# APRIL-ZJU/Ctrl-VIO

Measured on AMD Instinct MI355X. Metric: sliding-window solves/sec (10 KF, 200 lm, 2000 IMU), higher is better.
Workload: dtype f64; 1 GPU; config2: 10 KF / 200 landmarks / 2000 IMU sliding window (K = 24 knots, 814 reprojection blocks), <= 15 LM iterations (Ceres 1.14 trust region + projected line search); distinct_windows_per_gpu=64, streams_per_gpu=4, concurrent_solves_per_gpu=2

## Files before the change

### ctrl-vio_amd/csrc/kernels_solve.hpp

```cpp
#pragma once

namespace ctv {

__device__ __forceinline__ void begin_iteration(const Dev &d, int w, int *s_go) {
  Lm &lm = d.lm[w];
  if (threadIdx.x == 0) {
    int go = 0;
    if (!lm.status) {
      if (lm.ls_active) atomicAdd(d.n_active, 1);
      else if (lm.iter >= d.prm.max_iters) lm.status = 1 + 0;
      else if (lm.last_ok && __longlong_as_double((long long)lm.gmax_bits) <= d.prm.gtol) lm.status = 1 + 1;
      else if (lm.mu <= d.prm.min_radius) lm.status = 1 + 4;
      else {
        lm.iter += 1;
        lm.accept = 0; lm.step_valid = 0; lm.chol_fail = 0; lm.alpha = 1.0;
        atomicAdd(d.n_active, 1);
        go = 1;
      }
    }
    *s_go = go;
  }
  __syncthreads();
  if (!*s_go) return;
  const WinMeta &m = d.wins[w];
  const double mu = lm.mu;
  const double *Hd = d.HppS[lm.cur] + m.H0, *Hl = d.HllS[lm.cur] + m.lm0;
  for (int j = threadIdx.x; j < m.N; j += blockDim.x) {
    const bool act = d.active[m.u0 + j] != 0;
    const double c = d.cscale[m.u0 + j];
    const double h = (j < m.P) ? Hd[(long long)j * m.ldh + j] : Hl[j - m.P];
    const double sc = fmin(fmax(c * c * h, d.prm.min_diag), d.prm.max_diag);
    const double dd = act ? sc / (mu * c * c) : 0.0;
    d.dd[m.u0 + j] = dd;
    if (j >= m.P) {
      const int row = m.lm0 + d.lm_pos[m.lm0 + j - m.P];
      d.dinv[row] = (act && (h + dd) > 0.0) ? 1.0 / (h + dd) : 0.0;
      d.grs[row] = d.gS[lm.cur][m.u0 + j];
    }
  }
}
__global__ __launch_bounds__(256) void k_begin_iter(Dev d) {
  __shared__ int s_go;
  begin_iteration(d, blockIdx.x, &s_go);
}

__device__ __forceinline__ void tile_decode(int t, int &bi, int &bj) {
  bi = 0;
  while ((bi + 1) * (bi + 2) / 2 <= t) ++bi;
  bj = t - bi * (bi + 1) / 2;
}

struct SchurTiles {
  const int &K6, &P;
  __device__ bool nz_row(int b) const { return (16 * b < K6) || (P >= 16 * b && P - 1 < 16 * b + 16); }
  __device__ bool nz_col(int b) const { return (16 * b < K6) || (P - 1 >= 16 * b && P - 1 < 16 * b + 16); }
};

__device__ __forceinline__ void schur_row_range(const Dev &d, const WinMeta &m, int bi, int bj, int &lbeg, int &lend) {
  int rb = d.tl_beg[m.tr0 + bi], re = d.tl_end[m.tr0 + bi];
  if (16 * bi <= m.P && m.P < 16 * bi + 16) { rb = 0; re = m.Lobs; }
  lbeg = max(rb, d.tl_beg[m.tr0 + bj]);
  lend = min(re, d.tl_end[m.tr0 + bj]);
}

template <int NPRE, int NTQ> __global__ __launch_bounds__(512, NTQ <= 7 ? 4 : 2) void k_schur_window_f64(Dev d) {
  const int w = blockIdx.x;
  if (d.lm[w].status || d.lm[w].ls_active) return;
  const WinMeta &m = d.wins[w];
  const int P = m.P, L = m.L, ldw = m.ldw, u0 = m.u0, K6 = 6 * m.K, ldh = m.ldh;
  const int nt = ldw >> 4, ntile = nt * (nt + 1) / 2;
  extern __shared__ __attribute__((aligned(16))) double smd64[];
  const int ldl = ldw + 16;
  double *Wb = smd64;
  double *acts = Wb + 2 * 16 * ldl;
  double *ddv = acts + ldw;
  double *gv = ddv + ldw;
  double *dch = gv + ldw;
  int *tlist = reinterpret_cast<int *>(dch + 32);
  int &tcount = tlist[8 * NTQ];
  const int tid = threadIdx.x, wave = __builtin_amdgcn_readfirstlane(tid >> 6), lane = tid & 63, q4 = lane >> 4, l15 = lane & 15;
  const double *Wp = d.WS[d.lm[w].cur] + m.W0;
  const double *dinv = d.dinv + m.lm0, *gl = d.grs + m.lm0;
  for (int c = tid; c < ldw; c += 512) {
    const int cc = min(c, P - 1);
    acts[c] = (c < P && d.active[u0 + cc]) ? 1.0 : 0.0; ddv[c] = d.dd[u0 + cc]; gv[c] = d.gS[d.lm[w].cur][u0 + cc];
  }
  if (tid == 0) tcount = 0;
  const SchurTiles tiles{K6, P};
  __syncthreads();
  for (int t = tid; t < ntile; t += 512) {
    int ti, tj;
    tile_decode(t, ti, tj);
    if (tiles.nz_row(ti) && tiles.nz_col(tj)) { const int pos = atomicAdd(&tcount, 1); if (pos < 8 * NTQ) tlist[pos] = (ti << 8) | tj; }
  }
  const int nchunk = (m.Lobs + 15) >> 4, nel = 16 * ldl, NC = K6 + 2, nelc = 16 * NC;
  for (int e = tid; e < 2 * nel; e += 512) Wb[e] = 0.0;
  double pre[NPRE];
  double pre_d = 0.0;
  int pre_lc[NPRE];
  double keep[NPRE];
#pragma unroll
  for (int k = 0; k < NPRE; ++k) {
    const int e = min(tid + 512 * k, nelc - 1), cc = e % NC, c = cc < K6 ? cc : P - 1 + (cc - K6);
    pre_lc[k] = ((e / NC) << 16) | c | ((tid + 512 * k < nelc && c == P) ? 1 << 30 : 0);
  }
  auto fetch = [&](int ch) {
#pragma unroll
    for (int k = 0; k < NPRE; ++k) {
      const int l = min(16 * ch + ((pre_lc[k] >> 16) & 0xff), L - 1), c = pre_lc[k] & 0xffff;
      pre[k] = (c == P) ? gl[l] : Wp[(long long)l * ldw + c];
    }
    if (tid < 16) pre_d = dinv[min(16 * ch + tid, L - 1)];
  };
  auto stash = [&](int ch, int buf) {
#pragma unroll
    for (int k = 0; k < NPRE; ++k) {
      const int lr = (pre_lc[k] >> 16) & 0xff, c = pre_lc[k] & 0xffff;
      const bool lv = 16 * ch + lr < L && (pre_lc[k] >> 30) != 0;
      if (tid + 512 * k < nelc) Wb[buf * nel + lr * ldl + c] = lv ? pre[k] : 0.0;
    }
    if (tid < 16) dch[16 * buf + tid] = (16 * ch + tid < L) ? pre_d : 0.0;
  };
  __syncthreads();
#pragma unroll
  for (int k = 0; k < NPRE; ++k) keep[k] = acts[min(pre_lc[k] & 0xffff, ldw - 1)];
#pragma unroll
  for (int k = 0; k < NPRE; ++k) pre_lc[k] |= (tid + 512 * k < nelc && keep[k] != 0.0) ? 1 << 30 : 0;
  const int nact = min(tcount, 8 * NTQ);
  long long *dbg = (d.dbg && w == (d.nwin > 1000 ? 1000 : 0)) ? d.dbg + 96 : nullptr;
  int dbi = 0;
  CTV_STAMP(dbg, dbi, 30, tid == 0);
  int tij[NTQ];
#pragma unroll
  for (int q = 0; q < NTQ; ++q) tij[q] = __builtin_amdgcn_readfirstlane(tlist[(wave + 8 * q < nact) ? wave + 8 * q : min(wave, max(nact - 1, 0))]);
#pragma unroll
  for (int q = 0; q < NTQ; ++q) {
    int lb, le;
    schur_row_range(d, m, tij[q] >> 8, tij[q] & 255, lb, le);
    const bool real = wave + 8 * q < nact && le > lb;
    const int cb = real ? min(lb >> 4, 254) : 0, ce = real ? min((le + 15) >> 4, 255) : 0;
    tij[q] = __builtin_amdgcn_readfirstlane(tij[q] | (cb << 16) | (ce << 24));
  }
  const double *H = d.HppS[d.lm[w].cur] + m.H0;
  f64x4 acc[NTQ];
  const int opq = opaque_zero();
#pragma unroll
  for (int q = 0; q < NTQ; ++q) {
    const int tq = (tij[q] & 0xffff) + opq, jc = min(16 * (tq & 255) + l15, P - 1);
#pragma unroll
    for (int r = 0; r < 4; ++r) {
      const int ii = 16 * (tq >> 8) + q4 + 4 * r, ic = min(ii, P - 1);
      const double h = H[(unsigned)(ic * ldh + min(jc, ic))];
      acc[q][r] = ii < P ? -h : 0.0;
    }
  }
  if (nchunk > 0) { fetch(0); stash(0, 0); }
  __syncthreads();
  CTV_STAMP(dbg, dbi, 30, tid == 0);
  for (int ch = 0; ch < nchunk && nact > 0; ++ch) {
    const int buf = ch & 1;
    if (ch + 1 < nchunk) fetch(ch + 1);
    const double *B = Wb + buf * nel + q4 * ldl + l15;
    double dl[4];
#pragma unroll
    for (int s = 0; s < 4; ++s) dl[s] = dch[16 * buf + 4 * s + q4];
#pragma unroll
    for (int q = 0; q < NTQ; ++q) {
      { const int cb = (tij[q] >> 16) & 255, ce = (tij[q] >> 24) & 255; if (ch < cb || (ch >= ce && ce != 255)) continue; }
      double a[4], b[4];
#pragma unroll
      for (int s = 0; s < 4; ++s) {
        a[s] = B[4 * s * ldl + 16 * ((tij[q] >> 8) & 255)];
        b[s] = B[4 * s * ldl + 16 * (tij[q] & 255)];
      }
      __builtin_amdgcn_sched_barrier(0);
#pragma unroll
      for (int s = 0; s < 4; ++s) acc[q] = __builtin_amdgcn_mfma_f64_16x16x4f64(a[s], b[s] * dl[s], acc[q], 0, 0, 0);
      __builtin_amdgcn_sched_barrier(0);
    }
    if (ch + 1 < nchunk) stash(ch + 1, buf ^ 1);
    __syncthreads();
  }
  CTV_STAMP(dbg, dbi, 30, tid == 0);
  double *S = d.S + m.H0, *rhs = d.rhs + m.p0;
  auto pin = [](double &x) { asm volatile("" : "+v"(x)); };
  auto store_tile = [&](int ti, int tj, const double (&hs)[4], const double (&bs)[4]) {
    const int jj = 16 * tj + l15, jc = min(jj, P - 1);
    double a_j = acts[jc], dd_j = ddv[jc], g_j = gv[jc], a_i[4];
#pragma unroll
    for (int r = 0; r < 4; ++r) a_i[r] = acts[min(16 * ti + q4 + 4 * r, P - 1)];
    pin(a_j); pin(dd_j); pin(g_j);
#pragma unroll
    for (int r = 0; r < 4; ++r) pin(a_i[r]);
    const bool act_j = a_j != 0.0;
#pragma unroll
    for (int r = 0; r < 4; ++r) {
      const int ii = 16 * ti + q4 + 4 * r;
      if (ii < P && jj <= ii) {
        const bool on = a_i[r] != 0.0 && act_j;
        S[(long long)ii * ldh + jj] = on ? hs[r] + (ii == jj ? dd_j : 0.0) : (ii == jj ? 1.0 : 0.0);
      } else if (ii == P && jj < P) {
        rhs[jj] = act_j ? bs[r] - g_j : 0.0;
      }
    }
  };
#pragma unroll
  for (int q = 0; q < NTQ; ++q) {
    if (wave + 8 * q >= nact) continue;
    double hs[4], bs[4];
#pragma unroll
    for (int r = 0; r < 4; ++r) { hs[r] = -acc[q][r]; bs[r] = acc[q][r]; }
    store_tile((tij[q] >> 8) & 255, tij[q] & 255, hs, bs);
  }
  CTV_STAMP(dbg, dbi, 30, tid == 0);
  auto next_plain = [&](int t) {
    for (; t < ntile; t += 8) {
      int ti, tj;
      tile_decode(t, ti, tj);
      if (!(tiles.nz_row(ti) && tiles.nz_col(tj))) break;
    }
    return t;
  };
  if (d.schur_plain_in_H) {
    for (int c = tid; c < P; c += 512)
      if (!tiles.nz_col(c >> 4)) rhs[c] = acts[c] != 0.0 ? -gv[c] : 0.0;
  } else
  for (int tp = next_plain(wave); tp < ntile;) {
    int pi[4], pj[4];
#pragma unroll
    for (int u = 0; u < 4; ++u) {
      pi[u] = -1; pj[u] = 0;
      if (tp < ntile) { tile_decode(tp, pi[u], pj[u]); tp = next_plain(tp + 8); }
    }
    double hv[4][4];
#pragma unroll
    for (int u = 0; u < 4; ++u) {
      const int ti = max(pi[u], 0), jc = min(16 * pj[u] + l15, P - 1);
#pragma unroll
      for (int r = 0; r < 4; ++r) {
        const int ic = min(16 * ti + q4 + 4 * r, P - 1);
        hv[u][r] = H[(unsigned)(ic * ldh + min(jc, ic))];
      }
    }
    const double zero[4] = {0.0, 0.0, 0.0, 0.0};
#pragma unroll
    for (int u = 0; u < 4; ++u)
      if (pi[u] >= 0) store_tile(pi[u], pj[u], hv[u], zero);
  }
  CTV_STAMP(dbg, dbi, 30, tid == 0);
}

__global__ __launch_bounds__(64) void k_schur_tile_f64(Dev d, int ntile_max) {
  const int xcd = blockIdx.x & 7, slot = blockIdx.x >> 3;
  const int w = (slot / ntile_max) * 8 + xcd, tile = slot % ntile_max;
  if (w >= d.nwin) return;
  if (d.lm[w].status || d.lm[w].ls_active) return;
  const WinMeta &m = d.wins[w];
  const int P = m.P, L = m.L, ldw = m.ldw, u0 = m.u0, ldh = m.ldh;
  const int nt = P / 16 + 1;
  if (tile >= nt * (nt + 1) / 2) return;
  int bi, bj;
  tile_decode(tile, bi, bj);
  if (bj < d.env_first[m.tr0 + bi]) return;
  const int lane = threadIdx.x, q4 = lane >> 4, l15 = lane & 15;
  const int i = min(16 * bi + l15, ldw - 1), j = min(16 * bj + l15, ldw - 1);
  const bool rhs_lane = 16 * bi + l15 == P;
  const double ai = (16 * bi + l15 < P && d.active[u0 + min(i, P - 1)]) ? 1.0 : 0.0;
  const double aj = (16 * bj + l15 < P && d.active[u0 + min(j, P - 1)]) ? 1.0 : 0.0;
  const double *Wp = d.WS[d.lm[w].cur] + m.W0;
  const double *dinv = d.dinv + m.lm0, *gl = d.grs + m.lm0;
  int lbeg, lend;
  schur_row_range(d, m, bi, bj, lbeg, lend);
  f64x4 acc = {0.0, 0.0, 0.0, 0.0};
  for (int l0 = lbeg; l0 < lend; l0 += 16) {
    double wa[4], wb[4], dv[4], gv[4];
#pragma unroll
    for (int s = 0; s < 4; ++s) {
      const int lc = min(l0 + 4 * s + q4, L - 1);
      wa[s] = Wp[(long long)lc * ldw + i];
      wb[s] = Wp[(long long)lc * ldw + j];
      dv[s] = dinv[lc];
      gv[s] = gl[lc];
    }
#pragma unroll
    for (int s = 0; s < 4; ++s) wa[s] = rhs_lane ? gv[s] : wa[s] * ai;
#pragma unroll
    for (int s = 0; s < 4; ++s) {
      const bool lv = l0 + 4 * s + q4 < lend;
      acc = __builtin_amdgcn_mfma_f64_16x16x4f64(wa[s], lv ? wb[s] * aj * dv[s] : 0.0, acc, 0, 0, 0);
    }
  }
  double *S = d.S + m.H0, *rhs = d.rhs + m.p0;
  const double *H = d.HppS[d.lm[w].cur] + m.H0;
  const int jj = 16 * bj + l15, jc = min(jj, P - 1);
  const bool act_j = d.active[u0 + jc] != 0;
  const double dd_j = d.dd[u0 + jc], g_j = d.gS[d.lm[w].cur][u0 + jc];
  double hv[4];
  unsigned char act_i[4];
#pragma unroll
  for (int r = 0; r < 4; ++r) {
    const int ic = min(16 * bi + q4 + 4 * r, P - 1);
    act_i[r] = d.active[u0 + ic];
    hv[r] = H[(long long)ic * ldh + min(jc, ic)];
  }
#pragma unroll
  for (int r = 0; r < 4; ++r) {
    const int ii = 16 * bi + q4 + 4 * r;
    if (ii < P && jj <= ii) {
      const bool on = act_i[r] && act_j;
      S[(long long)ii * ldh + jj] = on ? hv[r] - acc[r] + (ii == jj ? dd_j : 0.0) : (ii == jj ? 1.0 : 0.0);
    } else if (ii == P && jj < P) {
      rhs[jj] = act_j ? acc[r] - g_j : 0.0;
    }
  }
}

__global__ __launch_bounds__(64) void k_schur_tile2_f64(Dev d, int nblk_max) {
  const int xcd = blockIdx.x & 7, slot = blockIdx.x >> 3;
  const int w = (slot / nblk_max) * 8 + xcd, blk = slot % nblk_max;
  if (w >= d.nwin) return;
  if (d.lm[w].status || d.lm[w].ls_active) return;
  const WinMeta &m = d.wins[w];
  const int P = m.P, L = m.L, ldw = m.ldw, u0 = m.u0, ldh = m.ldh;
  const int nt = P / 16 + 1, nb = (nt + 1) / 2;
  if (blk >= nb * (nb + 1) / 2) return;
  int Bi, Bj;
  tile_decode(blk, Bi, Bj);
  const int lane = threadIdx.x, q4 = lane >> 4, l15 = lane & 15;
  const int cur = d.lm[w].cur;
  const double *Wp = d.WS[cur] + m.W0;
  const double *dinv = d.dinv + m.lm0, *gl = d.grs + m.lm0;
  int ci[2], cj[2];
  bool rhs_lane[2];
  double ai[2], aj[2];
#pragma unroll
  for (int a = 0; a < 2; ++a) {
    const int bi = 2 * Bi + a, bj = 2 * Bj + a;
    ci[a] = min(16 * bi + l15, ldw - 1); cj[a] = min(16 * bj + l15, ldw - 1);
    rhs_lane[a] = 16 * bi + l15 == P;
    ai[a] = (16 * bi + l15 < P && d.active[u0 + min(ci[a], P - 1)]) ? 1.0 : 0.0;
    aj[a] = (16 * bj + l15 < P && d.active[u0 + min(cj[a], P - 1)]) ? 1.0 : 0.0;
  }
  bool live[2][2];
  int lbeg = L, lend = 0;
  bool any = false;
#pragma unroll
  for (int a = 0; a < 2; ++a)
#pragma unroll
    for (int b = 0; b < 2; ++b) {
      const int bi = 2 * Bi + a, bj = 2 * Bj + b;
      live[a][b] = bi < nt && bj <= bi && bj >= d.env_first[m.tr0 + min(bi, nt - 1)];
      if (live[a][b]) {
        any = true;
        int rb, re;
        schur_row_range(d, m, bi, bj, rb, re);
        if (re > rb) { lbeg = min(lbeg, rb); lend = max(lend, re); }
      }
    }
  if (!any) return;
  if (lend <= lbeg) { lbeg = 0; lend = 0; }
  f64x4 acc[2][2];
#pragma unroll
  for (int a = 0; a < 2; ++a)
#pragma unroll
    for (int b = 0; b < 2; ++b) acc[a][b] = f64x4{0.0, 0.0, 0.0, 0.0};
  struct Chunk { double wa[2][4], wb[2][4], dv[4], gv[4]; };
  auto fetch = [&](int l0, Chunk &c) {
#pragma unroll
    for (int s = 0; s < 4; ++s) {
      const int lc = max(0, min(l0 + 4 * s + q4, L - 1));
      const double *row = Wp + (long long)lc * ldw;
      c.wa[0][s] = row[ci[0]]; c.wa[1][s] = row[ci[1]];
      c.wb[0][s] = row[cj[0]]; c.wb[1][s] = row[cj[1]];
      c.dv[s] = dinv[lc];
      c.gv[s] = gl[lc];
    }
  };
  const bool upper = Bi != Bj;
  auto products = [&](int l0, const Chunk &c) {
#pragma unroll
    for (int s = 0; s < 4; ++s) {
      const bool lv = l0 + 4 * s + q4 < lend;
      const double dvs = lv ? c.dv[s] : 0.0;
      const double a0 = rhs_lane[0] ? c.gv[s] : c.wa[0][s] * ai[0], a1 = rhs_lane[1] ? c.gv[s] : c.wa[1][s] * ai[1];
      const double b0 = c.wb[0][s] * aj[0] * dvs, b1 = c.wb[1][s] * aj[1] * dvs;
      acc[0][0] = __builtin_amdgcn_mfma_f64_16x16x4f64(a0, b0, acc[0][0], 0, 0, 0);
      acc[1][0] = __builtin_amdgcn_mfma_f64_16x16x4f64(a1, b0, acc[1][0], 0, 0, 0);
      acc[1][1] = __builtin_amdgcn_mfma_f64_16x16x4f64(a1, b1, acc[1][1], 0, 0, 0);
      if (upper) acc[0][1] = __builtin_amdgcn_mfma_f64_16x16x4f64(a0, b1, acc[0][1], 0, 0, 0);
    }
  };
  if (L > 0 && lend > lbeg) {
    Chunk ca, cb;
    fetch(lbeg, ca);
    for (int l0 = lbeg; l0 < lend; l0 += 32) {
      fetch(l0 + 16, cb);
      __builtin_amdgcn_sched_barrier(0);
      products(l0, ca);
      __builtin_amdgcn_sched_barrier(0);
      fetch(l0 + 32, ca);
      __builtin_amdgcn_sched_barrier(0);
      if (l0 + 16 < lend) products(l0 + 16, cb);
      __builtin_amdgcn_sched_barrier(0);
    }
  }
  double *S = d.S + m.H0, *rhs = d.rhs + m.p0;
  const double *H = d.HppS[cur] + m.H0, *gp = d.gS[cur] + u0;
#pragma unroll
  for (int a = 0; a < 2; ++a)
#pragma unroll
    for (int b = 0; b < 2; ++b) {
      const int bi = 2 * Bi + a, bj = 2 * Bj + b;
      if (!live[a][b]) continue;
      const int jj = 16 * bj + l15, jc = min(jj, P - 1);
      const bool act_j = d.active[u0 + jc] != 0;
      const double dd_j = d.dd[u0 + jc], g_j = gp[jc];
      double hv[4];
      unsigned char av[4];
#pragma unroll
      for (int r = 0; r < 4; ++r) {
        const int ic = min(16 * bi + q4 + 4 * r, P - 1);
        hv[r] = H[(long long)ic * ldh + min(jc, ic)];
        av[r] = d.active[u0 + ic];
      }
      asm volatile("" : "+v"(hv[0]), "+v"(hv[1]), "+v"(hv[2]), "+v"(hv[3]));
#pragma unroll
      for (int r = 0; r < 4; ++r) {
        const int ii = 16 * bi + q4 + 4 * r;
        if (ii < P && jj <= ii) {
          const bool on = av[r] && act_j;
          S[(long long)ii * ldh + jj] = on ? hv[r] - acc[a][b][r] + (ii == jj ? dd_j : 0.0) : (ii == jj ? 1.0 : 0.0);
        } else if (ii == P && jj < P) {
          rhs[jj] = act_j ? acc[a][b][r] - g_j : 0.0;
        }
      }
    }
}


template <int C> __device__ __forceinline__ void chol_bcast_update(double &vc, double vj, int vj_lo, int vj_hi) {
  asm("v_readlane_b32 s96, %2, %4\n\tv_readlane_b32 s97, %3, %4\n\ts_nop 1\n\t"
      "v_fma_f64 %0, -%1, s[96:97], %0"
      : "+v"(vc)
      : "v"(vj), "v"(vj_lo), "v"(vj_hi), "n"(C)
      : "s96", "s97");
}
template <int C> __device__ __forceinline__ void chol_bcast_update_first(double &vc, double vj, int vj_lo, int vj_hi) {
  asm("s_nop 1\n\tv_readlane_b32 s96, %2, %4\n\tv_readlane_b32 s97, %3, %4\n\ts_nop 1\n\t"
      "v_fma_f64 %0, -%1, s[96:97], %0\n\ts_nop 1"
      : "+v"(vc)
      : "v"(vj), "v"(vj_lo), "v"(vj_hi), "n"(C)
      : "s96", "s97");
}
__device__ __forceinline__ double chol_pivot_rsqrt(double pj, int &bad) {
  const bool ok = (pj > 0.0) && isfinite(pj);
  if (!ok) bad = 1;
  const double ps = ok ? pj : 1.0;
  double di = __builtin_amdgcn_rsq(ps);
  const double hp = 0.5 * ps;
  di = di * (1.5 - hp * di * di);
  di = di * (1.5 - hp * di * di);
  return di;
}
template <int C> __device__ __forceinline__ void chol_bcast_update4(double &v0, double &v1, double &v2, double &v3, double vj, int vj_lo, int vj_hi) {
  asm("v_readlane_b32 s92, %5, %7\n\tv_readlane_b32 s93, %6, %7\n\t"
      "v_readlane_b32 s94, %5, %8\n\tv_readlane_b32 s95, %6, %8\n\t"
      "v_readlane_b32 s96, %5, %9\n\tv_readlane_b32 s97, %6, %9\n\t"
      "v_readlane_b32 s98, %5, %10\n\tv_readlane_b32 s99, %6, %10\n\t"
      "v_fma_f64 %0, -%4, s[92:93], %0\n\tv_fma_f64 %1, -%4, s[94:95], %1\n\t"
      "v_fma_f64 %2, -%4, s[96:97], %2\n\tv_fma_f64 %3, -%4, s[98:99], %3"
      : "+v"(v0), "+v"(v1), "+v"(v2), "+v"(v3)
      : "v"(vj), "v"(vj_lo), "v"(vj_hi), "n"(C), "n"(C + 1), "n"(C + 2), "n"(C + 3)
      : "s92", "s93", "s94", "s95", "s96", "s97", "s98", "s99");
}
template <int J, int C> __device__ __forceinline__ void chol_row_updates(double (&v)[32], int lo, int hi) {
  if constexpr (C + 3 <= 31) {
    chol_bcast_update4<C>(v[C], v[C + 1], v[C + 2], v[C + 3], v[J], lo, hi);
    chol_row_updates<J, C + 4>(v, lo, hi);
  } else if constexpr (C <= 31) {
    chol_bcast_update<C>(v[C], v[J], lo, hi);
// ... 952 lines not shown
```

### ctrl-vio_amd/csrc/kernels_visual.hpp

```cpp
#pragma once

namespace ctv {

__device__ __forceinline__ void vis_times(const WinMeta &m, long long t_rel, int row, double ld, int &s, double &u) {
  const long long ld_ns = (long long)(ld * 1e9);
  const long long tau = t_rel + (long long)row * ld_ns;
  s = (int)(tau / m.dt_ns);
  u = (double)(tau % m.dt_ns) / (double)m.dt_ns;
}

constexpr int AREC_LD = AREC + 1;
__device__ __forceinline__ void vis_anchor_body(const Dev &d, int mode, double *srec , int block) {
  const int a = block * 64 + threadIdx.x;
  bool run = false;
  if (a < d.Atot) run = lin_run(d.lm[d.a_win[a]], mode);
  const unsigned long long run_mask = __ballot(run);
  if (run_mask == 0) return;
  if (run) {
  const int w = d.a_win[a];
  const Lm &lm = d.lm[w];
  const WinMeta &m = d.wins[w];
  const bool jac = !lin_cost_only(lm, mode, d.prm);
  const bool at_cand = mode == LIN_SPEC;
  const double *quat = at_cand ? d.cquat : d.quat, *pos = at_cand ? d.cpos : d.pos, *rho = at_cand ? d.crho : d.rho, *ldp = at_cand ? d.cld : d.ld;
  int si;
  double ui;
  const int rowi = d.a_row[a];
  vis_times(m, d.a_t[a], rowi, ldp[w], si, ui);
  si = max(0, min(si, m.K - 4));
  SegConstLazy sc;
  seg_const_lazy(d.lkd + 3 * (m.knot0 + si), d.kjri + 9 * (m.knot0 + si), sc);
  double dmax = 0.0;
#pragma unroll
  for (int i = 0; i < 3; ++i) dmax = fmax(dmax, dot(sc.d[i], sc.d[i]));
  const bool small = __ballot(dmax >= 0.25) == 0ull;
  const double *qi = quat + 4 * (m.knot0 + si), *pi = pos + 3 * (m.knot0 + si);
  const Q4 q0 = qmk(qi[0], qi[1], qi[2], qi[3]);
  V3 p[4];
#pragma unroll
  for (int i = 0; i < 4; ++i) p[i] = mk(pi[3 * i], pi[3 * i + 1], pi[3 * i + 2]);
  const Q4 q_CI = qmk(m.q_CI[0], m.q_CI[1], m.q_CI[2], m.q_CI[3]);
  const V3 p_CI = mk(m.p_CI[0], m.p_CI[1], m.p_CI[2]);
  double *rec = srec + AREC_LD * threadIdx.x;
  if (!jac)
    for (int e = 0; e < AREC; ++e) rec[e] = 0.0;
  const double pix = d.a_obs[a], piy = d.a_obs[(size_t)d.Atot + a], d_inv = rho[m.lm0 + d.a_lm[a]];
  if (small) vis_anchor_eval<true>(q0, p, sc, ui, m.inv_dt, q_CI, p_CI, pix, piy, (double)rowi, d_inv, jac, rec);
  else vis_anchor_eval<false>(q0, p, sc, ui, m.inv_dt, q_CI, p_CI, pix, piy, (double)rowi, d_inv, jac, rec);
  d.a_s[a] = si;
  }
  lds_wave_sync();
  {
    const int lane = threadIdx.x;
    double *dst = d.arec + (size_t)(block * 64) * AREC;
    constexpr int HP = AREC / 2;
#pragma unroll 5
    for (int k = 0; k < HP; ++k) {
      const int i = k * 64 + lane, bl = i / HP, r = 2 * (i - bl * HP);
      VecN<double, 2> pr;
      pr.v[0] = srec[AREC_LD * bl + r];
      pr.v[1] = srec[AREC_LD * bl + r + 1];
      if ((run_mask >> bl) & 1ull) *reinterpret_cast<VecN<double, 2> *>(dst + (size_t)bl * AREC + r) = pr;
    }
  }
}
__global__ __launch_bounds__(64) void k_vis_anchor(Dev d, int mode) {
  __shared__ __attribute__((aligned(16))) double srec[64 * AREC_LD];
  vis_anchor_body(d, mode, srec, blockIdx.x);
}

constexpr int VT_LD = VT_ROWS + 1;
struct VisRecSink {
  double *J;
  __device__ __forceinline__ void put(int e, double v) { J[e] = v; }
};
struct VisNullSink {
  __device__ __forceinline__ void put(int, double) {}
};

constexpr int VIS_LDS_BYTES = 64 * VT_LD * 8;
__device__ __forceinline__ void vis_eval_body(const Dev &d, int mode, unsigned char *smt, long long *rowoff, int *rlm, int *rspan, int vblock) {
  const int v = vblock * 64 + threadIdx.x;
  const long long t_entry = d.dbg ? clock64() : 0ll;
  constexpr int LDS_BYTES = VIS_LDS_BYTES;
  double *wcs = reinterpret_cast<double *>(smt);
  const bool at_cand = mode == LIN_SPEC;
  const double *quat = at_cand ? d.cquat : d.quat, *pos = at_cand ? d.cpos : d.pos, *ldp = at_cand ? d.cld : d.ld;
  double c = 0.0;
  int ksj = 0, my_lm = -1, my_anc = -1;
  bool on = false, costed = false;
  const int wu = d.vb_win[vblock];
  const Lm &lmw = d.lm[wu];
  const WinMeta &m = d.wins[wu];
  if (!lin_run(lmw, mode)) return;
  const bool jac = !lin_cost_only(lmw, mode, d.prm);
  const int tgw = lin_target(lmw, mode);
  if (v < d.Vtot && d.v_win[v] >= 0) {
    {
      int sj;
      double uj;
      const int rowj = d.v_rowj[v];
      vis_times(m, d.v_tj[v], rowj, ldp[wu], sj, uj);
      sj = max(0, min(sj, m.K - 4));
      SegConstLazy scj;
      seg_const_lazy(d.lkd + 3 * (m.knot0 + sj), d.kjri + 9 * (m.knot0 + sj), scj);
      double dmax = 0.0;
#pragma unroll
      for (int i = 0; i < 3; ++i) dmax = fmax(dmax, dot(scj.d[i], scj.d[i]));
      const bool small = __ballot(dmax >= 0.25) == 0ull;
      const double *qj = quat + 4 * (m.knot0 + sj), *pj = pos + 3 * (m.knot0 + sj);
      const Q4 q0 = qmk(qj[0], qj[1], qj[2], qj[3]);
      V3 p[4];
#pragma unroll
      for (int i = 0; i < 4; ++i) p[i] = mk(pj[3 * i], pj[3 * i + 1], pj[3 * i + 2]);
      const int anc = d.v_anc[v];
      const double *rec = reinterpret_cast<const double *>(__builtin_assume_aligned(d.arec + (size_t)anc * AREC, 16));
      M3 RCIT;
      {
        const M3 R = q2R(qmk(m.q_CI[0], m.q_CI[1], m.q_CI[2], m.q_CI[3]));
#pragma unroll
        for (int a = 0; a < 3; ++a)
#pragma unroll
          for (int b = 0; b < 3; ++b) RCIT.m[3 * a + b] = R.m[3 * b + a];
      }
      const V3 p_CI = mk(m.p_CI[0], m.p_CI[1], m.p_CI[2]);
      const double pjx = d.v_obs[v], pjy = d.v_obs[(size_t)d.Vtot + v], ca = d.v_cauchy[v];
      double r[2];
      if (jac) {
        VisRecSink sink{wcs + VT_LD * threadIdx.x};
        on = true;
        my_lm = d.v_lm[v];
        my_anc = anc;
        if (small) c = vis_block_eval<true>(rec, q0, p, scj, uj, m.inv_dt, RCIT, p_CI, m.img_w, ca, pjx, pjy, (double)rowj, r, true, sink);
        else c = vis_block_eval<false>(rec, q0, p, scj, uj, m.inv_dt, RCIT, p_CI, m.img_w, ca, pjx, pjy, (double)rowj, r, true, sink);
        sink.J[VB_RES] = r[0]; sink.J[VB_RES + 1] = r[1];
        d.vsj[v] = sj;
        ksj = sj;
      } else {
        VisNullSink nsink;
        costed = true;
        c = vis_block_eval<false>(rec, q0, p, scj, uj, m.inv_dt, RCIT, p_CI, m.img_w, ca, pjx, pjy, (double)rowj, r, false, nsink);
      }
    }
  }
  {
    const int lane = threadIdx.x;
    const unsigned long long on_mask = __ballot(on);
    if (on_mask != 0 || __any(costed)) {
      double cs = c;
#pragma unroll
      for (int off = 32; off > 0; off >>= 1) cs += __shfl_xor(cs, off);
      if (lane == 0) d.vis_cost[vblock] = cs;
    }
    if (on_mask == 0) return;
    const int P = m.P, ldw = m.ldw, lm0 = m.lm0, u0 = m.u0;
    const long long W0 = m.W0;
    double *Wset = d.WS[tgw];
    double *Hllset = d.HllS[tgw], *gset = d.gS[tgw];
    long long *dbg = (d.dbg && vblock == 1000) ? d.dbg + 32 : nullptr;
    if (dbg && lane == 0) { dbg[-1] = t_entry; dbg[0] = clock64() + (long long)(c * 0); }
    lds_wave_sync();
    double wj[24], s6[6];
    {
      const double *Jl = wcs + VT_LD * lane;
      const double jr0 = Jl[VB_RHO], jr1 = Jl[VB_RHO + 1];
#pragma unroll
      for (int cc = 0; cc < 12; ++cc) wj[cc] = jr0 * Jl[VB_JROT + 2 * cc] + jr1 * Jl[VB_JROT + 2 * cc + 1];
#pragma unroll
      for (int b = 0; b < 3; ++b) s6[b] = jr0 * Jl[VB_AT + 2 * b] + jr1 * Jl[VB_AT + 2 * b + 1];
#pragma unroll
      for (int k = 0; k < 4; ++k) {
        const double cp1 = Jl[VB_CP1 + k];
#pragma unroll
        for (int b = 0; b < 3; ++b) wj[12 + 3 * k + b] = -(cp1 * s6[b]);
      }
      s6[3] = jr0 * Jl[VB_LD] + jr1 * Jl[VB_LD + 1];
      s6[4] = jr0 * jr0 + jr1 * jr1;
      s6[5] = jr0 * Jl[VB_RES] + jr1 * Jl[VB_RES + 1];
    }
    double hg[40];
    int ksi, my_row, my_klo, my_khi;
    {
      const double *rec = reinterpret_cast<const double *>(__builtin_assume_aligned(d.arec + (size_t)max(my_anc, 0) * AREC, 16));
#pragma unroll
      for (int e = 0; e < 40; ++e) hg[e] = rec[AR_GR + e];
      ksi = d.a_s[max(my_anc, 0)];
      my_row = d.lm_pos[lm0 + max(my_lm, 0)];
      my_klo = d.lm_klo[lm0 + my_row]; my_khi = d.lm_khi[lm0 + my_row];
    }
    const int prev_lm = __shfl_up(my_lm, 1), prev_anc = __shfl_up(my_anc, 1);
    const bool head = on && (lane == 0 || prev_lm != my_lm), head_a = on && (lane == 0 || prev_anc != my_anc);
    const unsigned long long heads = __ballot(head), heads_a = __ballot(head_a);
    const int ord = __popcll(heads & ((2ull << lane) - 1ull)) - 1;
    const int nlm = __popcll(heads);
    const int ha = 63 - __clzll((long long)(heads_a & ((2ull << lane) - 1ull)));
    int maxlen = on ? lane - ha + 1 : 0;
#pragma unroll
    for (int off = 32; off > 0; off >>= 1) maxlen = max(maxlen, __shfl_xor(maxlen, off));
    maxlen = __builtin_amdgcn_readfirstlane(maxlen);
    for (int off = 1; off < maxlen; off <<= 1) {
      const int oh = __shfl_down(on ? ha : -1, off);
      const bool take = on && (lane + off < 64) && oh == ha;
#pragma unroll
      for (int cc = 0; cc < 6; ++cc) { const double o = __shfl_down(s6[cc], off); s6[cc] += take ? o : 0.0; }
    }
    if (dbg && lane == 0) dbg[1] = clock64() + (long long)(s6[0] * 0);
    {
      double *dst = d.Jt + (size_t)(vblock * 64) * VT_ROWS;
      constexpr int HP = VT_ROWS / 2;
#pragma unroll 4
      for (int k = 0; k < HP; ++k) {
        const int i = k * 64 + lane, bl = i / HP, r = 2 * (i - bl * HP);
        VecN<double, 2> pr;
        pr.v[0] = wcs[VT_LD * bl + r];
        pr.v[1] = wcs[VT_LD * bl + r + 1];
        if ((on_mask >> bl) & 1ull) *reinterpret_cast<VecN<double, 2> *>(dst + (size_t)bl * VT_ROWS + r) = pr;
      }
    }
    if (dbg && lane == 0) dbg[2] = clock64();
    double wi[24];
#pragma unroll
    for (int k = 0; k < 4; ++k)
#pragma unroll
      for (int b = 0; b < 3; ++b) {
        const int cc = 3 * k + b;
        wi[cc] = s6[0] * hg[3 * cc] + s6[1] * hg[3 * cc + 1] + s6[2] * hg[3 * cc + 2];
        wi[12 + cc] = hg[36 + k] * s6[b];
      }
    double *rows = reinterpret_cast<double *>(smt);
    const int SPW = d.max_span6;
    const int RS = SPW + 3;
    const int NR = max(1, min(nlm, ((int)(LDS_BYTES / 8) - 1) / RS));
    if (head) { rowoff[ord] = W0 + (long long)my_row * ldw; rlm[ord] = my_lm; rspan[ord] = (my_klo << 16) | max(my_khi - my_klo + 1, 0); }
    int ri = ksi - my_klo, rj = ksj - my_klo;
    if (on && (rj < 0 || ksj + 3 > my_khi || (head_a && (ri < 0 || ksi + 3 > my_khi)))) atomicAdd(d.span_viol, 1);
    ri = max(0, min(ri, SPW / 6 - 4)); rj = max(0, min(rj, SPW / 6 - 4));
    lds_wave_sync();
    for (int c0 = 0; c0 < nlm; c0 += NR) {
      const int nr = min(NR, nlm - c0);
      for (int i = 2 * lane; i < nr * RS; i += 128) *reinterpret_cast<VecN<double, 2> *>(rows + i) = VecN<double, 2>{{0.0, 0.0}};
      lds_wave_sync();
      if (on && ord >= c0 && ord < c0 + nr) {
        double *row = rows + (size_t)(ord - c0) * RS;
        if (head_a) {
#pragma unroll
          for (int k = 0; k < 4; ++k)
#pragma unroll
            for (int b = 0; b < 3; ++b) {
              atomicAdd(&row[6 * (ri + k) + b], wi[3 * k + b]);
              atomicAdd(&row[6 * (ri + k) + 3 + b], wi[12 + 3 * k + b]);
            }
          atomicAdd(&row[SPW], s6[3]);
          atomicAdd(&row[SPW + 1], s6[4]);
          atomicAdd(&row[SPW + 2], s6[5]);
        }
#pragma unroll
        for (int k = 0; k < 4; ++k)
#pragma unroll
          for (int b = 0; b < 3; ++b) {
            atomicAdd(&row[6 * (rj + k) + b], wj[3 * k + b]);
            atomicAdd(&row[6 * (rj + k) + 3 + b], wj[12 + 3 * k + b]);
          }
      }
      lds_wave_sync();
      if (dbg && lane == 0) dbg[3 + 2 * (c0 / NR)] = clock64();
      {
        for (int rb = 0; rb < nr; rb += 4) {
          const int q = rb + (lane >> 4);
          if (q < nr) {
            const int sp = rspan[c0 + q], k0 = sp >> 16, npair = 3 * (sp & 0xffff);
            double *Wr = Wset + rowoff[c0 + q] + 6 * k0;
            const double *row = rows + (size_t)q * RS;
            for (int cp = lane & 15; cp < npair; cp += 16) {
              VecN<double, 2> rv;
              rv.v[0] = row[2 * cp]; rv.v[1] = row[2 * cp + 1];
              *reinterpret_cast<VecN<double, 2> *>(Wr + 2 * cp) = rv;
            }
          }
        }
        if (lane < nr) {
          const double *row = rows + (size_t)lane * RS;
          const int l = rlm[c0 + lane];
          Wset[rowoff[c0 + lane] + P - 1] = row[SPW];
          Hllset[lm0 + l] = row[SPW + 1];
          gset[u0 + P + l] = row[SPW + 2];
        }
      }
      lds_wave_sync();
      if (dbg && lane == 0) { dbg[4 + 2 * (c0 / NR)] = clock64(); dbg[10] = nlm * 1000000ll; dbg[11] = NR * 1000; }
    }
  }
}

__global__ __launch_bounds__(64) __attribute__((amdgpu_waves_per_eu(2))) void k_vis_eval(Dev d, int mode) {
  __shared__ __attribute__((aligned(16))) unsigned char smt[VIS_LDS_BYTES];
  __shared__ long long rowoff[64];
  __shared__ int rlm[64], rspan[64];
  vis_eval_body(d, mode, smt, rowoff, rlm, rspan, blockIdx.x);
}

__global__ __launch_bounds__(64) __attribute__((amdgpu_waves_per_eu(1, 1))) void k_linearize_f64(Dev d, int mode, int general_only, int zero_mode) {
  static_assert(VIS_LDS_BYTES >= (72 * 33 + 64) * 8, "the IMU rows use the head of the visual body's LDS buffer");
  __shared__ __attribute__((aligned(32))) unsigned char smt[VIS_LDS_BYTES];
  __shared__ long long rowoff[64];
  __shared__ int rlm[64], rspan[64];
  if ((int)blockIdx.x < d.Gtot) {
    if (!general_only) imu_linearize_f64_fast(d, mode, reinterpret_cast<double *>(smt), blockIdx.x, d.Gtot, zero_mode);
  } else vis_eval_body(d, mode, smt, rowoff, rlm, rspan, blockIdx.x - d.Gtot);
}

}
```

Before: 46820 solves/s.

## Swizzle visual Jacobian LDS layout and skip MFMA substeps outside Schur row range

The visual eval kernel drops the padded VT_LD stride for the per-thread Jacobian staging buffer. It uses an XOR swizzle instead to avoid LDS bank conflicts, and packs the rowoff/rlm/rspan arrays into the tail of the same LDS buffer, shrinking the shared-memory footprint. The rowoff/rlm/rspan writes move after the wave sync, because they now alias the staging buffer. In the Schur complement kernel, the row-range bounds are tracked at 4-element granularity instead of 16-element chunks, so individual MFMA k-steps outside a tile's nonzero range are skipped. This adds per-step branching and reduces the row-buffer capacity (NR) slightly.

Result: faster. 47360 solves/s, median of 6 (+1.2%).

```diff
diff --git a/ctrl-vio_amd/csrc/kernels_solve.hpp b/ctrl-vio_amd/csrc/kernels_solve.hpp
--- a/ctrl-vio_amd/csrc/kernels_solve.hpp
+++ b/ctrl-vio_amd/csrc/kernels_solve.hpp
@@ -138,8 +138,8 @@
     int lb, le;
     schur_row_range(d, m, tij[q] >> 8, tij[q] & 255, lb, le);
     const bool real = wave + 8 * q < nact && le > lb;
-    const int cb = real ? min(lb >> 4, 254) : 0, ce = real ? min((le + 15) >> 4, 255) : 0;
-    tij[q] = __builtin_amdgcn_readfirstlane(tij[q] | (cb << 16) | (ce << 24));
+    const int kb = real ? min(lb >> 2, 254) : 0, ke = real ? min((le + 3) >> 2, 255) : 0;
+    tij[q] = __builtin_amdgcn_readfirstlane(tij[q] | (kb << 16) | (ke << 24));
   }
   const double *H = d.HppS[d.lm[w].cur] + m.H0;
   f64x4 acc[NTQ];
@@ -166,7 +166,9 @@
     for (int s = 0; s < 4; ++s) dl[s] = dch[16 * buf + 4 * s + q4];
 #pragma unroll
     for (int q = 0; q < NTQ; ++q) {
-      { const int cb = (tij[q] >> 16) & 255, ce = (tij[q] >> 24) & 255; if (ch < cb || (ch >= ce && ce != 255)) continue; }
+      const int kb = (tij[q] >> 16) & 255, ke = (tij[q] >> 24) & 255;
+      const int s0 = max(kb - 4 * ch, 0), s1 = ke == 255 ? 4 : min(ke - 4 * ch, 4);
+      if (s0 >= s1) continue;
       double a[4], b[4];
 #pragma unroll
       for (int s = 0; s < 4; ++s) {
@@ -175,7 +177,8 @@
       }
       __builtin_amdgcn_sched_barrier(0);
 #pragma unroll
-      for (int s = 0; s < 4; ++s) acc[q] = __builtin_amdgcn_mfma_f64_16x16x4f64(a[s], b[s] * dl[s], acc[q], 0, 0, 0);
+      for (int s = 0; s < 4; ++s)
+        if (s >= s0 && s < s1) acc[q] = __builtin_amdgcn_mfma_f64_16x16x4f64(a[s], b[s] * dl[s], acc[q], 0, 0, 0);
       __builtin_amdgcn_sched_barrier(0);
     }
     if (ch + 1 < nchunk) stash(ch + 1, buf ^ 1);
diff --git a/ctrl-vio_amd/csrc/kernels_visual.hpp b/ctrl-vio_amd/csrc/kernels_visual.hpp
--- a/ctrl-vio_amd/csrc/kernels_visual.hpp
+++ b/ctrl-vio_amd/csrc/kernels_visual.hpp
@@ -69,20 +69,24 @@
   vis_anchor_body(d, mode, srec, blockIdx.x);
 }
 
-constexpr int VT_LD = VT_ROWS + 1;
+__device__ __forceinline__ int vt_at(int l, int e) { return VT_ROWS * l + (e ^ ((l >> 2) & 7)); }
 struct VisRecSink {
-  double *J;
-  __device__ __forceinline__ void put(int e, double v) { J[e] = v; }
+  double *wcs;
+  int l;
+  __device__ __forceinline__ void put(int e, double v) { wcs[vt_at(l, e)] = v; }
 };
 struct VisNullSink {
   __device__ __forceinline__ void put(int, double) {}
 };
 
-constexpr int VIS_LDS_BYTES = 64 * VT_LD * 8;
-__device__ __forceinline__ void vis_eval_body(const Dev &d, int mode, unsigned char *smt, long long *rowoff, int *rlm, int *rspan, int vblock) {
+constexpr int VIS_LDS_BYTES = 64 * VT_ROWS * 8;
+constexpr int VIS_ROW_BYTES = VIS_LDS_BYTES - 64 * 16;
+__device__ __forceinline__ void vis_eval_body(const Dev &d, int mode, unsigned char *smt, int vblock) {
   const int v = vblock * 64 + threadIdx.x;
   const long long t_entry = d.dbg ? clock64() : 0ll;
-  constexpr int LDS_BYTES = VIS_LDS_BYTES;
+  constexpr int LDS_BYTES = VIS_ROW_BYTES;
+  long long *rowoff = reinterpret_cast<long long *>(smt + VIS_ROW_BYTES);
+  int *rlm = reinterpret_cast<int *>(rowoff + 64), *rspan = rlm + 64;
   double *wcs = reinterpret_cast<double *>(smt);
   const bool at_cand = mode == LIN_SPEC;
   const double *quat = at_cand ? d.cquat : d.quat, *pos = at_cand ? d.cpos : d.pos, *ldp = at_cand ? d.cld : d.ld;
@@ -127,13 +131,13 @@
       const double pjx = d.v_obs[v], pjy = d.v_obs[(size_t)d.Vtot + v], ca = d.v_cauchy[v];
       double r[2];
       if (jac) {
-        VisRecSink sink{wcs + VT_LD * threadIdx.x};
+        VisRecSink sink{wcs, (int)threadIdx.x};
         on = true;
         my_lm = d.v_lm[v];
         my_anc = anc;
         if (small) c = vis_block_eval<true>(rec, q0, p, scj, uj, m.inv_dt, RCIT, p_CI, m.img_w, ca, pjx, pjy, (double)rowj, r, true, sink);
         else c = vis_block_eval<false>(rec, q0, p, scj, uj, m.inv_dt, RCIT, p_CI, m.img_w, ca, pjx, pjy, (double)rowj, r, true, sink);
-        sink.J[VB_RES] = r[0]; sink.J[VB_RES + 1] = r[1];
+        sink.put(VB_RES, r[0]); sink.put(VB_RES + 1, r[1]);
         d.vsj[v] = sj;
         ksj = sj;
       } else {
@@ -162,21 +166,21 @@
     lds_wave_sync();
     double wj[24], s6[6];
     {
-      const double *Jl = wcs + VT_LD * lane;
-      const double jr0 = Jl[VB_RHO], jr1 = Jl[VB_RHO + 1];
-#pragma unroll
-      for (int cc = 0; cc < 12; ++cc) wj[cc] = jr0 * Jl[VB_JROT + 2 * cc] + jr1 * Jl[VB_JROT + 2 * cc + 1];
-#pragma unroll
-      for (int b = 0; b < 3; ++b) s6[b] = jr0 * Jl[VB_AT + 2 * b] + jr1 * Jl[VB_AT + 2 * b + 1];
+      auto Jl = [&](int e) { return wcs[vt_at(lane, e)]; };
+      const double jr0 = Jl(VB_RHO), jr1 = Jl(VB_RHO + 1);
+#pragma unroll
+      for (int cc = 0; cc < 12; ++cc) wj[cc] = jr0 * Jl(VB_JROT + 2 * cc) + jr1 * Jl(VB_JROT + 2 * cc + 1);
+#pragma unroll
+      for (int b = 0; b < 3; ++b) s6[b] = jr0 * Jl(VB_AT + 2 * b) + jr1 * Jl(VB_AT + 2 * b + 1);
 #pragma unroll
       for (int k = 0; k < 4; ++k) {
-        const double cp1 = Jl[VB_CP1 + k];
+        const double cp1 = Jl(VB_CP1 + k);
 #pragma unroll
         for (int b = 0; b < 3; ++b) wj[12 + 3 * k + b] = -(cp1 * s6[b]);
       }
-      s6[3] = jr0 * Jl[VB_LD] + jr1 * Jl[VB_LD + 1];
+      s6[3] = jr0 * Jl(VB_LD) + jr1 * Jl(VB_LD + 1);
       s6[4] = jr0 * jr0 + jr1 * jr1;
-      s6[5] = jr0 * Jl[VB_RES] + jr1 * Jl[VB_RES + 1];
+      s6[5] = jr0 * Jl(VB_RES) + jr1 * Jl(VB_RES + 1);
     }
     double hg[40];
     int ksi, my_row, my_klo, my_khi;
@@ -211,9 +215,11 @@
 #pragma unroll 4
       for (int k = 0; k < HP; ++k) {
         const int i = k * 64 + lane, bl = i / HP, r = 2 * (i - bl * HP);
+        const int sw = (bl >> 2) & 7;
+        const VecN<double, 2> pp = *reinterpret_cast<const VecN<double, 2> *>(wcs + VT_ROWS * bl + (r ^ (sw & 6)));
         VecN<double, 2> pr;
-        pr.v[0] = wcs[VT_LD * bl + r];
-        pr.v[1] = wcs[VT_LD * bl + r + 1];
+        pr.v[0] = (sw & 1) ? pp.v[1] : pp.v[0];
+        pr.v[1] = (sw & 1) ? pp.v[0] : pp.v[1];
         if ((on_mask >> bl) & 1ull) *reinterpret_cast<VecN<double, 2> *>(dst + (size_t)bl * VT_ROWS + r) = pr;
       }
     }
@@ -231,11 +237,11 @@
     const int SPW = d.max_span6;
     const int RS = SPW + 3;
     const int NR = max(1, min(nlm, ((int)(LDS_BYTES / 8) - 1) / RS));
-    if (head) { rowoff[ord] = W0 + (long long)my_row * ldw; rlm[ord] = my_lm; rspan[ord] = (my_klo << 16) | max(my_khi - my_klo + 1, 0); }
     int ri = ksi - my_klo, rj = ksj - my_klo;
     if (on && (rj < 0 || ksj + 3 > my_khi || (head_a && (ri < 0 || ksi + 3 > my_khi)))) atomicAdd(d.span_viol, 1);
     ri = max(0, min(ri, SPW / 6 - 4)); rj = max(0, min(rj, SPW / 6 - 4));
     lds_wave_sync();
+    if (head) { rowoff[ord] = W0 + (long long)my_row * ldw; rlm[ord] = my_lm; rspan[ord] = (my_klo << 16) | max(my_khi - my_klo + 1, 0); }
     for (int c0 = 0; c0 < nlm; c0 += NR) {
       const int nr = min(NR, nlm - c0);
       for (int i = 2 * lane; i < nr * RS; i += 128) *reinterpret_cast<VecN<double, 2> *>(rows + i) = VecN<double, 2>{{0.0, 0.0}};
@@ -294,19 +300,15 @@
 
 __global__ __launch_bounds__(64) __attribute__((amdgpu_waves_per_eu(2))) void k_vis_eval(Dev d, int mode) {
   __shared__ __attribute__((aligned(16))) unsigned char smt[VIS_LDS_BYTES];
-  __shared__ long long rowoff[64];
-  __shared__ int rlm[64], rspan[64];
-  vis_eval_body(d, mode, smt, rowoff, rlm, rspan, blockIdx.x);
+  vis_eval_body(d, mode, smt, blockIdx.x);
 }
 
 __global__ __launch_bounds__(64) __attribute__((amdgpu_waves_per_eu(1, 1))) void k_linearize_f64(Dev d, int mode, int general_only, int zero_mode) {
   static_assert(VIS_LDS_BYTES >= (72 * 33 + 64) * 8, "the IMU rows use the head of the visual body's LDS buffer");
   __shared__ __attribute__((aligned(32))) unsigned char smt[VIS_LDS_BYTES];
-  __shared__ long long rowoff[64];
-  __shared__ int rlm[64], rspan[64];
   if ((int)blockIdx.x < d.Gtot) {
     if (!general_only) imu_linearize_f64_fast(d, mode, reinterpret_cast<double *>(smt), blockIdx.x, d.Gtot, zero_mode);
-  } else vis_eval_body(d, mode, smt, rowoff, rlm, rspan, blockIdx.x - d.Gtot);
-}
-
-}
+  } else vis_eval_body(d, mode, smt, blockIdx.x - d.Gtot);
+}
+
+}
```
